# mheinz757/AgglomerationMultigrid1D

Measured on AMD Instinct MI355X. Metric: fine_level_dof_updates_per_s_per_vcycle, higher is better.
Workload: dtype f64; 1 GPU; config 3/4 hierarchy: V(3,3) cycle, alpha=2/3, DG p=3 n=2^24 -> AggDG pAgg=1 4:1 -> 2:1 -> 2:1 (4 levels), uniform mesh, Neumann/Dirichlet, CDir=1000n (north-star 1-vs-8-GPU size; config 3's own 2^22 in config3_2p22); fine_dofs=67108864, nPre=3, nPost=3, parallelism=single GPU

## Files before the change

agglomerationmultigrid1d_amd/_lib.py:

```python
import ctypes
import os
from ctypes import POINTER, c_char_p, c_double, c_int, c_int32, c_int64, c_void_p

_HERE = os.path.dirname(os.path.abspath(__file__))
LIB_PATH = os.environ.get("AGGMG_HIP_LIB") or os.path.join(_HERE, "libaggmg_hip.so")

AGGMG_OK = 0
ERR_ARGUMENT, ERR_DIMENSION, ERR_SINGULAR, ERR_HIP, ERR_UNSUPPORTED = -1, -2, -3, -4, -5
OP_STIFFNESS, OP_TRANSFER = 0, 1
OPT_SYMMETRIC_PACKING = 1
OPT_COARSE_CHUNK_LOG2 = 2
OPT_DETECT_CHAIN = 3
OPT_PAIR_LEVELS = 4
OPT_MG_CHECKPOINT = 5
OPT_SYMMETRIC_RESIDUAL = 6
OPT_OPERATOR_DICTIONARY = 7
OPT_ELEMENT_THREADS = 8
OPT_PAIR_ELEMENT_THREADS = 9
OPT_REPLAY_PRESMOOTH = 10
OPT_PATCH_MULTI = 11
OPT_CHAIN_MULTI = 12
PROFILE_NTAGS = 256
KIND_FUSED_DOWN, KIND_FUSED_UP, KIND_SMOOTH, KIND_RESIDUAL, KIND_RESTRICT, KIND_PROLONG, \
    KIND_JACOBI, KIND_BLOCK_APPLY, KIND_COARSE, KIND_FUSED_MID = range(10)
KIND_REPLAY_DOWN, KIND_REPLAY_UP = 10, 11
KIND_NAMES = ["fused_down", "fused_up", "smooth", "residual", "restrict", "prolong", "jacobi",
              "block_apply", "coarse", "fused_mid"]
COARSE_HOST_BANDED, COARSE_DEVICE_CR, COARSE_AUTO, COARSE_EXTERNAL = 0, 1, 2, 3
COARSE_DEVICE_CHAIN = 4
RESTRICT_EXPLICIT, RESTRICT_PRECONDITIONED = 0, 1
RESTRICT_PRECONDITIONED_MAX_ELEMS = 1 << 21
LEVEL_GENERIC, LEVEL_FUSED_BTD, LEVEL_FUSED_CHAIN, LEVEL_COARSEST = 0, 1, 2, 3
MAX_SWEEP_WEIGHTS = 8
FGMRES_MAX_RESTART = 64
RCCL_ID_BYTES = 128
DIST_X0_GHOSTS_VALID, DIST_OVERLAP_NEXT, DIST_GRAPH = 1, 2, 4
# ... 31 lines not shown
                              UnsupportedError)}

_P = c_void_p
_PD = POINTER(c_double)
SYMBOLS = {
    "aggmg_create": (c_int, [c_int, POINTER(_P)]),
    "aggmg_destroy": (c_int, [_P]),
    "aggmg_last_error": (c_char_p, [_P]),
    "aggmg_set_stream": (c_int, [_P, _P]),
    "aggmg_reset_stream": (c_int, [_P]),
    "aggmg_synchronize": (c_int, [_P]),
    "aggmg_set_option": (c_int, [_P, c_int, c_int]),
    "aggmg_element_thread_launches": (c_int, [_P, POINTER(c_int64)]),
    "aggmg_pair_element_thread_launches": (c_int, [_P, POINTER(c_int64)]),
    "aggmg_replay_launches": (c_int, [_P, POINTER(c_int64)]),
    "aggmg_patch_multi_launches": (c_int, [_P, POINTER(c_int64)]),
    "aggmg_chain_multi_launches": (c_int, [_P, POINTER(c_int64)]),
    "aggmg_chain_multi_tile_plan": (c_int, [c_int, c_int, c_int, c_int, c_int, POINTER(c_int), POINTER(c_int), POINTER(c_int),
                                            POINTER(c_int), POINTER(c_int)]),
    "aggmg_dev_alloc": (c_int, [_P, c_int64, POINTER(_P)]),
    "aggmg_dev_free": (c_int, [_P, _P]),
    "aggmg_memcpy_h2d": (c_int, [_P, _P, _P, c_int64]),
    "aggmg_memcpy_d2h": (c_int, [_P, _P, _P, c_int64]),
    "aggmg_csc_upload": (c_int, [_P, c_int64, c_int64, POINTER(c_int64), POINTER(c_int64), _PD,
                                 c_int, c_int, POINTER(_P)]),
    "aggmg_op_free": (c_int, [_P, _P]),
    "aggmg_op_shape": (c_int, [_P, _P, POINTER(c_int64), POINTER(c_int64), POINTER(c_int64)]),
    "aggmg_op_download": (c_int, [_P, _P, c_int, POINTER(c_int32), POINTER(c_int32), _PD]),
    "aggmg_op_release_host": (c_int, [_P, _P]),
    "aggmg_bd_sp_apply": (c_int, [_P, _P, _P, c_int, POINTER(_P)]),
# ... 156 lines not shown
```

agglomerationmultigrid1d_amd/api.py:

```python
import ctypes

import numpy as np
import scipy.sparse as sp
import scipy.sparse.linalg as spla

from . import _lib
from ._lib import (ArgumentError, DimensionMismatch, check)

_PD = ctypes.POINTER(ctypes.c_double)
_PI64 = ctypes.POINTER(ctypes.c_int64)


def _f64(x):
    return np.ascontiguousarray(x, dtype=np.float64)


def _pd(a):
    return a.ctypes.data_as(_PD)


def device_memory():
    n, b = ctypes.c_int64(), ctypes.c_int64()
    check(_lib.load().aggmg_debug_device_memory(ctypes.byref(n), ctypes.byref(b)), None)
    return n.value, b.value
# ... 31 lines not shown

    def element_thread_launches(self):
        n = ctypes.c_int64(0)
        self.check(self.lib.aggmg_element_thread_launches(self.handle, ctypes.byref(n)))
        return int(n.value)

    def pair_element_thread_launches(self):
        n = ctypes.c_int64(0)
        self.check(self.lib.aggmg_pair_element_thread_launches(self.handle, ctypes.byref(n)))
        return int(n.value)

    def replay_launches(self):
        n = ctypes.c_int64(0)
        self.check(self.lib.aggmg_replay_launches(self.handle, ctypes.byref(n)))
        return int(n.value)

    def patch_multi_launches(self):
        n = ctypes.c_int64(0)
        self.check(self.lib.aggmg_patch_multi_launches(self.handle, ctypes.byref(n)))
        return int(n.value)

    def chain_multi_launches(self):
        n = ctypes.c_int64(0)
        self.check(self.lib.aggmg_chain_multi_launches(self.handle, ctypes.byref(n)))
        return int(n.value)

    def option(self, option, default):
        return self.__dict__.get("_options", {}).get(int(option), default)

    def set_stream(self, hip_stream):
# ... 1526 lines not shown
```

agglomerationmultigrid1d_amd/csrc/aggmg_hip.hip:

```cpp
#include "internal.hpp"
#include "multi_kernels.hpp"
#include "multi_solve_kernels.hpp"
#include "pair_kernels.hpp"
#include "patch_kernels.hpp"
#include "patch_multi_kernels.hpp"
#include "elem_kernels.hpp"
#include "pair_elem_kernels.hpp"
#include "krylov_kernels.hpp"
#include "host_gmres.hpp"
#include "host_gmres_cols.hpp"

extern "C" const char* aggmg_version(void) { return "aggmg_hip 0.1 gfx950 fp64"; }

extern "C" int aggmg_debug_device_memory(int64_t* live_allocations, int64_t* live_bytes) {
  if (live_allocations) *live_allocations = DevMemLive::allocations.load();
  if (live_bytes) *live_bytes = DevMemLive::bytes.load();
  return AGGMG_OK;
}

extern "C" int aggmg_create(int device_id, aggmg_ctx** out) {
  if (!out) return fail(nullptr, AGGMG_ERR_ARGUMENT, "aggmg_create: out is NULL");
  *out = nullptr;
  int ndev = 0;
  hipError_t e = hipGetDeviceCount(&ndev);
// ... 133 lines not shown
    case AGGMG_OPT_SYMMETRIC_RESIDUAL:
      ctx->sym_residual = value != 0;
      return AGGMG_OK;
    case AGGMG_OPT_OPERATOR_DICTIONARY:
      ctx->op_dict = value != 0;
      return AGGMG_OK;
    case AGGMG_OPT_ELEMENT_THREADS:
      ctx->elem_threads = value != 0;
      return AGGMG_OK;
    case AGGMG_OPT_PAIR_ELEMENT_THREADS:
      ctx->pair_elem_threads = value != 0;
      return AGGMG_OK;
    case AGGMG_OPT_REPLAY_PRESMOOTH:
      ctx->replay_presmooth = value != 0;
      return AGGMG_OK;
    case AGGMG_OPT_PATCH_MULTI:
      ctx->patch_multi = value != 0;
      return AGGMG_OK;
    case AGGMG_OPT_CHAIN_MULTI:
      ctx->chain_multi = value != 0;
      return AGGMG_OK;
  }
  return fail(ctx, AGGMG_ERR_ARGUMENT, "aggmg_set_option: unknown option");
}

extern "C" int aggmg_synchronize(aggmg_ctx* ctx) {
  if (!ctx) return AGGMG_ERR_ARGUMENT;
  HIPCHK(hipStreamSynchronize(ctx->stream));
  return AGGMG_OK;
}
// ... 327 lines not shown
  static const int max_shift = env_int("AGGMG_AGG_ALIGN", 1) ? 8 : -1;
  return (!t.rho && t.maxagg >= 1 && t.maxagg - 1 <= max_shift) ? t.maxagg - 1 : -1;
}
static void xfer_out(FusedArgs& a, const TransferBtd& t) {
  a.lf1_out = t.lf1;
  a.mc_out = t.mc;
  a.rho_out = t.rho;
  a.par_out = t.rho ? nullptr : t.parent;
  a.first_out = t.rho ? nullptr : t.first;
  a.nec_out = t.nec;
  a.agg_shift = xfer_agg_shift(t);
}

struct FusedLaunch : FusedArgs {
  SweepWeights wts;
};

static bool elem_thread_args(const aggmg_ctx* ctx, const FusedArgs& a, bool chk, int sel_mode) {
  return ctx->elem_threads && a.lv.cls && a.lv.bsym && !a.gs && !chk && a.nsweeps >= 1 && sel_mode == 0 && !a.r_out &&
         !a.par_in && !a.par_out && !a.ld_out && (!a.lf_in || a.mc_in == 2) && (!a.lf_out || a.mc_out == 2) &&
         (!a.do_residual || a.lf_out);
}

template <int M, bool CMP>
static int launch_btd_t(aggmg_ctx* ctx, FusedLaunch a, int halo, const TileSel& sel, CgtChk* chk_io) {
  using T = BtdTile<M, CMP>;
  const bool vr = (a.lf_out || a.ld_out) && a.par_out;
  const int align = ((a.lf_out || a.ld_out) && !vr) ? a.rho_out : 1;
  if (a.gs) halo += a.nsweeps;
  if (vr && (sel.mode == 1 || sel.mode == 2))
    return fail(ctx, AGGMG_ERR_UNSUPPORTED, "tile selection on a level with agglomerates of different sizes");
  const bool chk = a.chk_part != nullptr;
  bool elem = false;
  if constexpr (M == 4 && CMP)
    elem = elem_thread_args(ctx, a, chk, sel.mode) && fused_tile_plan(kElemThreads, halo, align, vr, a.agg_shift).owned > 0;
  const FusedTilePlan plan = fused_tile_plan(elem ? kElemThreads : T::TE, halo, align, vr, a.agg_shift);
// ... 25 lines not shown
  const size_t lds = (size_t)2 * (T::TE + 2) * M * sizeof(double) +
                     (chk ? ((size_t)2 * (T::NT / 64) + (CMP ? (size_t)T::NT * T::NS * (M + 1) : 0)) * sizeof(double) : 0);
  constexpr bool kGrp = (CMP && (M == 2 || M == 4 || M == 8)) || (!CMP && (M == 2 || M == 4));
  const bool sym = kGrp && a.lv.bsym;
  constexpr bool kSres = kGrp && CMP && M <= 4;
  const bool sres = kSres && a.lv.dup && !a.gs && !chk && a.do_residual && (a.r_out || a.lf_out);
  auto go = [&](auto kern) {
    hipLaunchKernelGGL(kern, dim3((unsigned)ntiles), dim3(T::NT), lds, ctx->stream, static_cast<const FusedArgs&>(a), a.wts);
  };
  if constexpr (kGrp && CMP && M <= 4) {
    if (sym && a.lv.cls) {
      if (a.gs || chk) return fail(ctx, AGGMG_ERR_UNSUPPORTED, "internal: dictionary launch of a Gauss-Seidel / checkpoint variant");
      if (a.par_in || a.par_out || a.ld_out || (a.lf_in && a.mc_in != 2) || (a.lf_out && a.mc_out != 2))
        return fail(ctx, AGGMG_ERR_UNSUPPORTED, "internal: dictionary launch with a transfer the variant does not index by class");
      if constexpr (M == 4) {
        if (elem) {
          auto go_elem = [&](auto kern) {
            hipLaunchKernelGGL(kern, dim3((unsigned)ntiles), dim3(kElemThreads), elem_lds_bytes<M>(), ctx->stream,
                               static_cast<const FusedArgs&>(a), a.wts);
          };
          if (sres)
            go_elem(btd_elem_dict_kernel<M, true>);
          else
            go_elem(btd_elem_dict_kernel<M, false>);
          HIPCHK(hipGetLastError());
          ++ctx->elem_launches;
          return AGGMG_OK;
        }
      }
      if (sres)
// ... 93 lines not shown
  a.uc = uc;
  xfer_in(a, *l.tb);
}
static bool restrict_with_ld(const aggmg_hier* h, const Level& l) {
  return l.tb->ld && h->restriction == AGGMG_RESTRICT_PRECONDITIONED;
}
static void fused_descent(FusedArgs& a, const aggmg_hier* h, const Level& l, double* rc) {
  a.do_residual = 1;
  if (restrict_with_ld(h, l))
    a.ld_out = l.tb->ld;
  else
    a.lf_out = l.tb->lf;
  a.rc_out = rc;
  xfer_out(a, *l.tb);
}
static void fused_dictionary(FusedArgs& a, const Level& l) {
  const DictDev* d = l.dict.get();
  if (!d || a.gs || a.chk_part || a.ld_out || a.par_in || a.par_out || !a.lv.bsym) return;
  if ((a.lf_in && a.mc_in != 2) || (a.lf_out && a.mc_out != 2)) return;
  a.lv.bsym = d->bsym;
  a.lv.qrow = d->qrow;
  a.lv.qmir = d->qmir;
  a.lv.dup = d->dup;
  a.lv.corr = d->corr;
  a.lv.scol = d->scol;
  a.lv.dblk = d->dblk;
  a.lv.cls = d->cls;
  if (a.lf_in) (d->lf_unit ? a.lf1_in : a.lf_in) = d->lf;
  if (a.lf_out) (d->lf_unit ? a.lf1_out : a.lf_out) = d->lf;
}
static void fused_chk(FusedArgs& a, const CgtChk& c) {
  a.chk_sweep = c.sweep;
  a.chk_stride = c.stride;
  a.chk_final = c.final;
  a.chk_exact = c.exact;
  a.chk_part = c.part;
}

static int btd_max_sweeps(const BtdDev& b, int extra) {
  const int te = btd_tile_elems(b);
  int s = std::min(8, te / 8) - extra;
  return std::max(1, s);
// ... 1651 lines not shown
  return AGGMG_OK;
}

extern "C" int aggmg_element_thread_launches(aggmg_ctx* ctx, int64_t* count) {
  if (!ctx || !count) return fail(ctx, AGGMG_ERR_ARGUMENT, "aggmg_element_thread_launches: NULL argument");
  *count = ctx->elem_launches;
  return AGGMG_OK;
}

extern "C" int aggmg_pair_element_thread_launches(aggmg_ctx* ctx, int64_t* count) {
  if (!ctx || !count) return fail(ctx, AGGMG_ERR_ARGUMENT, "aggmg_pair_element_thread_launches: NULL argument");
  *count = ctx->pair_elem_launches;
  return AGGMG_OK;
}

extern "C" int aggmg_replay_launches(aggmg_ctx* ctx, int64_t* count) {
  if (!ctx || !count) return fail(ctx, AGGMG_ERR_ARGUMENT, "aggmg_replay_launches: NULL argument");
  *count = ctx->replay_launches;
  return AGGMG_OK;
}

extern "C" int aggmg_hier_level_dictionary(aggmg_ctx* ctx, const aggmg_hier* h, int level, int* nclasses) {
  if (!ctx || !h || !nclasses) return fail(ctx, AGGMG_ERR_ARGUMENT, "aggmg_hier_level_dictionary: NULL argument");
  if (level < 0 || level >= (int)h->lv.size()) return fail(ctx, AGGMG_ERR_ARGUMENT, "aggmg_hier_level_dictionary: level out of range");
  const Level& l = h->lv[level];
  *nclasses = l.dict ? l.dict->nclasses : (l.cdict ? l.cdict->nclasses : (l.pdict ? l.pdict->nclasses : 0));
  return AGGMG_OK;
}

extern "C" int aggmg_hier_set_sweep_weights(aggmg_ctx* ctx, aggmg_hier* h, int level, const double* pre, int npre,
// ... 152 lines not shown
  return true;
}
static int btd_replay_up(aggmg_ctx* ctx, aggmg_hier* h, const double* x0, const double* b, int nPre, int nPost, double alpha,
                         double* dst) {
  FusedLaunch a = replay_up_args(h, x0, b, nPre, nPost, alpha, dst);
  const FusedTilePlan plan = fused_tile_plan(kElemThreads, nPre + nPost, 1, false, a.agg_shift);
  if (plan.owned <= 0) return fail(ctx, AGGMG_ERR_UNSUPPORTED, "internal: replayed ascent without a tile");
  a.agg_shift = plan.agg_shift;
  a.owned = plan.owned;
  a.halo_left = plan.halo_left;
  const TileSubset sub = fused_tile_subset(a.lv.ne, plan.owned, 0, 0, 0);
  a.tile_split = sub.split;
  a.tile_skip = sub.skip;
  if (sub.ntiles == 0) return AGGMG_OK;
  ProfScope ps(ctx, AGGMG_KIND_FUSED_UP, 0);
  hipLaunchKernelGGL(btd_elem_replay_up_kernel<4>, dim3((unsigned)sub.ntiles), dim3(kElemThreads), elem_lds_bytes<4>(), ctx->stream,
                     static_cast<const FusedArgs&>(a), a.wts, nPre);
  HIPCHK(hipGetLastError());
  ++ctx->elem_launches;
  ++ctx->replay_launches;
  return AGGMG_OK;
}

static bool patch_transfer_ok(const Level& l, int residual, const TransferBtd* tout) {
  if (!l.tb) return false;
  const BtdDev& B = *l.S->patch->btd;
  TileQuery q;
  q.launch = kTileFused;
  q.te = btd_tile_elems(B);
  q.halo = residual;
  if (tout) {
    q.var_agg = tout->rho == 0;
    q.align = tout->rho ? tout->rho : 1;
    q.agg_shift = xfer_agg_shift(*tout);
// ... 2395 lines not shown
```

agglomerationmultigrid1d_amd/csrc/elem_kernels.hpp:

```cpp
#pragma once
#include <type_traits>

#include "kernels.hpp"

namespace aggmg {

typedef double elem_v2d __attribute__((ext_vector_type(2)));
__device__ __forceinline__ void elem_ld2(const double* p, double& x, double& y) {
  const elem_v2d v = *reinterpret_cast<const elem_v2d*>(p);
  x = v.x;
  y = v.y;
}
template <int M>
__host__ __device__ constexpr int elem_tri(int i, int j) {
  return i * M - (i * (i - 1)) / 2 + (j - i);
}
template <int M>
__device__ __forceinline__ double elem_sym_row_apply(const double (&tri)[M * (M + 1) / 2], int i, const double (&v)[M]) {
  double acc = 0.0;
#pragma unroll
  for (int j = 0; j < M; ++j) acc = __fma_rn(tri[i < j ? elem_tri<M>(i, j) : elem_tri<M>(j, i)], v[j], acc);
  return acc;
}
__device__ __forceinline__ void elem_group_dot4(const double (&a)[4], const double (&b)[4], double& lo, double& hi) {
// ... 367 lines not shown
    double* const op = a.u_out + e0 * M + (unsigned)(x * M);
#pragma unroll
    for (int j = 0; j < M; j += 2) {
      elem_v2d v;
      v.x = uu[j];
      v.y = uu[j + 1];
#if AGGMG_NT & 2
      __builtin_nontemporal_store(v, reinterpret_cast<elem_v2d*>(op + j));
#else
      *reinterpret_cast<elem_v2d*>(op + j) = v;
#endif
    }
  }
}

}
```

agglomerationmultigrid1d_amd/csrc/host_plan.hpp:

```cpp
#pragma once
#include <algorithm>
#include <cstddef>
#include <cstdint>
#include <vector>

namespace aggmg {

constexpr int kCrTailRows = 4096;
constexpr int kCrMaxLevels = 40;
constexpr int kCrMaxStageLevels = 12;
constexpr int kCrMaxSteps = 8;

struct CrStagePlan {
  int l0 = 0, q = 0;
  int64_t n_in = 0, n_out = 0;
  int nsteps = 0;
  int step_a[kCrMaxSteps + 1] = {0};
  int lds_off[kCrMaxSteps + 1] = {0}, lds_xoff[kCrMaxSteps + 1] = {0};
  int lds_total = 0;
  int stack_stride = 0;
  int64_t mid_off[kCrMaxSteps + 1] = {0};
  int64_t mid_total = 0;
};

// ... 409 lines not shown
  int64_t rm = W[0];
  for (int k = 0; k < nl - 1; ++k) {
    if (ratio[k] < 1) return false;
    pu[k] = std::min(rm, W[k]) - dist_sweep_reach(kind[k], nPre, k > 0);
    if (pu[k] < 1) return false;
    rm = (pu[k] - 1) / ratio[k];
  }
  int64_t v = W[nl - 1];
  for (int k = nl - 2; k >= 0; --k) {
    v = std::min(pu[k], ratio[k] * v) - dist_sweep_reach(kind[k], nPost, false);
    if (v < 0) return false;
  }
  return true;
}

}
```

agglomerationmultigrid1d_amd/csrc/internal.hpp:

```cpp
#pragma once
#include "../../include/aggmg_hip.h"

#include <hip/hip_runtime.h>

#include <algorithm>
#include <array>
#include <atomic>
#include <chrono>
#include <cmath>
#include <cstdio>
#include <cstdlib>
#include <cstring>
#include <memory>
#include <string>
#include <type_traits>
#include <vector>

#include "kernels.hpp"
#include "cr_kernels.hpp"
#include "cgt_kernels.hpp"

using namespace aggmg;

struct aggmg_ctx;
// ... 28 lines not shown
  int device = 0;
  hipStream_t own_stream = nullptr;
  hipStream_t stream = nullptr;
  std::string err;
  bool sym_packing = true;
  int cr_max_q = 12;
  bool detect_chain = true;
  bool mg_checkpoint = [] { const char* e = std::getenv("AGGMG_MG_CHECKPOINT"); return !(e && e[0] == '0'); }();
  bool pair_levels = [] { const char* e = std::getenv("AGGMG_PAIR"); return !(e && e[0] == '0'); }();
  bool sym_residual = [] { const char* e = std::getenv("AGGMG_SYM_RESIDUAL"); return !(e && e[0] == '0'); }();
  bool op_dict = [] { const char* e = std::getenv("AGGMG_OP_DICT"); return !(e && e[0] == '0'); }();
  bool elem_threads = [] { const char* e = std::getenv("AGGMG_ELEM_THREADS"); return !(e && e[0] == '0'); }();
  int64_t elem_launches = 0;
  bool pair_elem_threads = [] { const char* e = std::getenv("AGGMG_PAIR_ELEM_THREADS"); return !(e && e[0] == '0'); }();
  int64_t pair_elem_launches = 0;
  bool replay_presmooth = [] { const char* e = std::getenv("AGGMG_REPLAY_PRESMOOTH"); return !(e && e[0] == '0'); }();
  int64_t replay_launches = 0;
  bool patch_multi = [] { const char* e = std::getenv("AGGMG_PATCH_MULTI"); return e && e[0] == '1'; }();
  int64_t patch_multi_launches = 0;
  bool chain_multi = [] { const char* e = std::getenv("AGGMG_CHAIN_MULTI"); return e && e[0] == '1'; }();
  int64_t chain_multi_launches = 0;
  int profiling = 0;
  std::vector<ProfEvent> prof;
  std::vector<hipEvent_t> ev_pool;
  WorkVectors<kScratchSlots> scratch;
  WorkVectors<kSolvSlots> solv;
  DevArray<double> solv_part, solv_sc;
  DevArray<double> cols_part, cols_sc;
  DevArray<int> cols_map;
  int64_t cols_cap = 0;
// ... 123 lines not shown
  DevArray<double> lf;
  DevArray<double> lf1;
  DevArray<double> ld;
  DevArray<int32_t> parent;
  DevArray<int32_t> first;
  int maxagg = 0;
};

struct DictDev {
  int nclasses = 0;
  DevArray<uint16_t> cls;
  DevArray<double> bsym, qrow, qmir, dup, scol, dblk;
  DevArray<uint32_t> corr;
  DevArray<double> lf;
  bool lf_unit = false;
};

struct PairDictDev {
  int nclasses = 0;
  DevArray<uint16_t> cls;
  DevArray<double> bsym, sup, sback, sub, dblk;
  DevArray<double> lf;
  bool lf_unit = false;
  DevArray<double> rec;
};

struct TransferCgt {
  int type = 0, mc = 0, rho = 1;
  int64_t nec = 0;
  DevArray<double> l, lp;
// ... 255 lines not shown
```

agglomerationmultigrid1d_amd/csrc/setup.hip:

```cpp
#include <functional>

#include <hipcub/hipcub.hpp>

#include "internal.hpp"
#include "setup_kernels.hpp"
#include "pair_elem_kernels.hpp"

namespace {

inline unsigned grid_for(int64_t n) { return (unsigned)((n + kSetupThreads - 1) / kSetupThreads); }

struct Flags {
  DevArray<int> d;
  int n = 0;
  int init(aggmg_ctx* ctx, int count) {
    n = count;
    return d.alloc(ctx, count, true);
  }
  int read(aggmg_ctx* ctx, int* host) {
    HIPCHK(hipMemcpyAsync(host, d, n * sizeof(int), hipMemcpyDeviceToHost, ctx->stream));
    HIPCHK(hipStreamSynchronize(ctx->stream));
    return AGGMG_OK;
  }
  int clear(aggmg_ctx* ctx) {
// ... 539 lines not shown
  const int T = m * (m + 1) / 2;
  auto d = std::make_unique<DictDev>();
  d->lf_unit = t.lf1 != nullptr;
  DictFields F(b.ne);
  F.add(b.bsym, &d->bsym, T);
  F.add(b.qrow, &d->qrow, m);
  F.add(b.qrow, &d->qmir, m, true);
  if (b.dup) {
    F.add(b.dup, &d->dup, T);
    F.add(b.corr, &d->corr, m);
  }
  F.add(b.scol, &d->scol, m);
  F.add(b.dblk, &d->dblk, m * m);
  F.add(t.lf1 ? t.lf1 : t.lf, &d->lf, m * (t.lf1 ? 1 : 2));
  CHECK(dict_build(ctx, F, &d->cls, &d->nclasses));
  if (d->nclasses > 0) *out = std::move(d);
  return AGGMG_OK;
}

int setup_pair_dictionary(aggmg_ctx* ctx, const BtdDev& b, const TransferBtd& t, std::unique_ptr<PairDictDev>* out) {
  out->reset();
  const int m = b.m;
  if (!(!b.cmp && m == 2 && b.bsym && b.sup && b.sub && b.dblk) || b.ne < 1) return AGGMG_OK;
  if (!(t.rho > 0 && t.mc == 2 && t.lf)) return AGGMG_OK;
  auto d = std::make_unique<PairDictDev>();
  d->lf_unit = t.lf1 != nullptr;
  DictFields F(b.ne);
  F.add(b.bsym, &d->bsym, m * (m + 1) / 2);
  F.add(b.sup, &d->sup, m * m);
  F.add(b.sup, &d->sback, m * m, true);
// ... 623 lines not shown
```

include/aggmg_hip.h:

```cpp
#ifndef AGGMG_HIP_H
#define AGGMG_HIP_H

#include <stdint.h>

#ifdef __cplusplus
extern "C" {
#endif

#define AGGMG_OK 0
#define AGGMG_ERR_ARGUMENT (-1)
#define AGGMG_ERR_DIMENSION (-2)
#define AGGMG_ERR_SINGULAR (-3)
#define AGGMG_ERR_HIP (-4)
#define AGGMG_ERR_UNSUPPORTED (-5)

typedef struct aggmg_ctx aggmg_ctx;
typedef struct aggmg_op aggmg_op;
typedef struct aggmg_smoother aggmg_smoother;
typedef struct aggmg_hier aggmg_hier;

int aggmg_create(int device_id, aggmg_ctx** out);
int aggmg_destroy(aggmg_ctx* ctx);
const char* aggmg_last_error(aggmg_ctx* ctx);
int aggmg_set_stream(aggmg_ctx* ctx, void* hip_stream);
int aggmg_reset_stream(aggmg_ctx* ctx);
int aggmg_synchronize(aggmg_ctx* ctx);
#define AGGMG_OPT_SYMMETRIC_PACKING 1
#define AGGMG_OPT_COARSE_CHUNK_LOG2 2
#define AGGMG_OPT_DETECT_CHAIN 3
#define AGGMG_OPT_PAIR_LEVELS 4
#define AGGMG_OPT_MG_CHECKPOINT 5
#define AGGMG_OPT_SYMMETRIC_RESIDUAL 6
#define AGGMG_OPT_OPERATOR_DICTIONARY 7
#define AGGMG_OPT_ELEMENT_THREADS 8
#define AGGMG_OPT_PAIR_ELEMENT_THREADS 9
#define AGGMG_OPT_REPLAY_PRESMOOTH 10
#define AGGMG_OPT_PATCH_MULTI 11
#define AGGMG_OPT_CHAIN_MULTI 12
int aggmg_set_option(aggmg_ctx* ctx, int option, int value);
int aggmg_element_thread_launches(aggmg_ctx* ctx, int64_t* count);
int aggmg_pair_element_thread_launches(aggmg_ctx* ctx, int64_t* count);
int aggmg_replay_launches(aggmg_ctx* ctx, int64_t* count);
int aggmg_patch_multi_launches(aggmg_ctx* ctx, int64_t* count);
int aggmg_chain_multi_launches(aggmg_ctx* ctx, int64_t* count);
int aggmg_chain_multi_tile_plan(int m, int nsweeps, int restrict_kind, int rho, int kb, int* tile_blocks, int* owned,
                                int* halo_left, int* halo_right, int* max_sweeps);
int aggmg_dev_alloc(aggmg_ctx* ctx, int64_t nbytes, void** out);
int aggmg_dev_free(aggmg_ctx* ctx, void* ptr);
int aggmg_memcpy_h2d(aggmg_ctx* ctx, void* dst_dev, const void* src_host, int64_t nbytes);
int aggmg_memcpy_d2h(aggmg_ctx* ctx, void* dst_host, const void* src_dev, int64_t nbytes);
int aggmg_host_register(aggmg_ctx* ctx, void* ptr, int64_t nbytes);
int aggmg_host_unregister(aggmg_ctx* ctx, void* ptr);
int aggmg_host_alloc(aggmg_ctx* ctx, int64_t nbytes, void** out);
int aggmg_host_free(aggmg_ctx* ctx, void* ptr);
// ... 243 lines not shown
```

Measured before the change: 467.7 billion DoF-updates/s.

## Stage per-class element records in LDS for element-thread fused kernels

```diff
diff --git a/agglomerationmultigrid1d_amd/_lib.py b/agglomerationmultigrid1d_amd/_lib.py
--- a/agglomerationmultigrid1d_amd/_lib.py
+++ b/agglomerationmultigrid1d_amd/_lib.py
@@ -20,6 +20,7 @@
 OPT_REPLAY_PRESMOOTH = 10
 OPT_PATCH_MULTI = 11
 OPT_CHAIN_MULTI = 12
+OPT_ELEMENT_RECORDS_LDS = 13
 PROFILE_NTAGS = 256
 KIND_FUSED_DOWN, KIND_FUSED_UP, KIND_SMOOTH, KIND_RESIDUAL, KIND_RESTRICT, KIND_PROLONG, \
     KIND_JACOBI, KIND_BLOCK_APPLY, KIND_COARSE, KIND_FUSED_MID = range(10)
@@ -81,6 +82,9 @@
     "aggmg_element_thread_launches": (c_int, [_P, POINTER(c_int64)]),
     "aggmg_pair_element_thread_launches": (c_int, [_P, POINTER(c_int64)]),
     "aggmg_replay_launches": (c_int, [_P, POINTER(c_int64)]),
+    "aggmg_element_record_lds_launches": (c_int, [_P, POINTER(c_int64)]),
+    "aggmg_element_record_lds_cap": (c_int, [_P, POINTER(c_int), POINTER(c_int)]),
+    "aggmg_element_record_pack": (c_int, [c_int, _P, _P, _P, _P, _P, _P, c_int, _P, POINTER(c_int)]),
     "aggmg_patch_multi_launches": (c_int, [_P, POINTER(c_int64)]),
     "aggmg_chain_multi_launches": (c_int, [_P, POINTER(c_int64)]),
     "aggmg_chain_multi_tile_plan": (c_int, [c_int, c_int, c_int, c_int, c_int, POINTER(c_int), POINTER(c_int), POINTER(c_int),
diff --git a/agglomerationmultigrid1d_amd/api.py b/agglomerationmultigrid1d_amd/api.py
--- a/agglomerationmultigrid1d_amd/api.py
+++ b/agglomerationmultigrid1d_amd/api.py
@@ -69,6 +69,16 @@
         n = ctypes.c_int64(0)
         self.check(self.lib.aggmg_replay_launches(self.handle, ctypes.byref(n)))
         return int(n.value)
+
+    def element_record_lds_launches(self):
+        n = ctypes.c_int64(0)
+        self.check(self.lib.aggmg_element_record_lds_launches(self.handle, ctypes.byref(n)))
+        return int(n.value)
+
+    def element_record_lds_cap(self):
+        c, m = ctypes.c_int(0), ctypes.c_int(0)
+        self.check(self.lib.aggmg_element_record_lds_cap(self.handle, ctypes.byref(c), ctypes.byref(m)))
+        return int(c.value), int(m.value)
 
     def patch_multi_launches(self):
         n = ctypes.c_int64(0)
diff --git a/agglomerationmultigrid1d_amd/csrc/aggmg_hip.hip b/agglomerationmultigrid1d_amd/csrc/aggmg_hip.hip
--- a/agglomerationmultigrid1d_amd/csrc/aggmg_hip.hip
+++ b/agglomerationmultigrid1d_amd/csrc/aggmg_hip.hip
@@ -171,6 +171,11 @@
     case AGGMG_OPT_REPLAY_PRESMOOTH:
       ctx->replay_presmooth = value != 0;
       return AGGMG_OK;
+    case AGGMG_OPT_ELEMENT_RECORDS_LDS:
+      if (value < 0 || value > kElemRecMaxClasses)
+        return fail(ctx, AGGMG_ERR_ARGUMENT, "aggmg_set_option: AGGMG_OPT_ELEMENT_RECORDS_LDS takes 0 .. " + std::to_string(kElemRecMaxClasses));
+      ctx->elem_rec_cap = value;
+      return AGGMG_OK;
     case AGGMG_OPT_PATCH_MULTI:
       ctx->patch_multi = value != 0;
       return AGGMG_OK;
@@ -528,12 +533,16 @@
 
 struct FusedLaunch : FusedArgs {
   SweepWeights wts;
+  ElemRecTab rec = {nullptr, 0};
 };
 
 static bool elem_thread_args(const aggmg_ctx* ctx, const FusedArgs& a, bool chk, int sel_mode) {
   return ctx->elem_threads && a.lv.cls && a.lv.bsym && !a.gs && !chk && a.nsweeps >= 1 && sel_mode == 0 && !a.r_out &&
          !a.par_in && !a.par_out && !a.ld_out && (!a.lf_in || a.mc_in == 2) && (!a.lf_out || a.mc_out == 2) &&
          (!a.do_residual || a.lf_out);
+}
+static bool elem_record_args(const aggmg_ctx* ctx, const FusedLaunch& a) {
+  return a.rec.rec && a.rec.nclasses >= 1 && a.rec.nclasses <= ctx->elem_rec_cap && (!a.do_residual || (a.lv.dup && a.lv.corr));
 }
 
 template <int M, bool CMP>
@@ -589,6 +598,20 @@
       if (a.par_in || a.par_out || a.ld_out || (a.lf_in && a.mc_in != 2) || (a.lf_out && a.mc_out != 2))
         return fail(ctx, AGGMG_ERR_UNSUPPORTED, "internal: dictionary launch with a transfer the variant does not index by class");
       if constexpr (M == 4) {
+        if (elem && elem_record_args(ctx, a)) {
+          auto go_rec = [&](auto kern) {
+            hipLaunchKernelGGL(kern, dim3((unsigned)ntiles), dim3(kElemThreads), elem_rec_lds_bytes<M>(a.rec.nclasses), ctx->stream,
+                               static_cast<const FusedArgs&>(a), a.wts, a.rec);
+          };
+          if (a.do_residual)
+            go_rec(btd_elem_rec_kernel<M, true>);
+          else
+            go_rec(btd_elem_rec_kernel<M, false>);
+          HIPCHK(hipGetLastError());
+          ++ctx->elem_launches;
+          ++ctx->elem_rec_launches;
+          return AGGMG_OK;
+        }
         if (elem) {
           auto go_elem = [&](auto kern) {
             hipLaunchKernelGGL(kern, dim3((unsigned)ntiles), dim3(kElemThreads), elem_lds_bytes<M>(), ctx->stream,
@@ -712,7 +735,7 @@
   a.rc_out = rc;
   xfer_out(a, *l.tb);
 }
-static void fused_dictionary(FusedArgs& a, const Level& l) {
+static void fused_dictionary(FusedLaunch& a, const Level& l) {
   const DictDev* d = l.dict.get();
   if (!d || a.gs || a.chk_part || a.ld_out || a.par_in || a.par_out || !a.lv.bsym) return;
   if ((a.lf_in && a.mc_in != 2) || (a.lf_out && a.mc_out != 2)) return;
@@ -724,6 +747,7 @@
   a.lv.scol = d->scol;
   a.lv.dblk = d->dblk;
   a.lv.cls = d->cls;
+  if (d->rec) a.rec = ElemRecTab{d->rec, d->nclasses};
   if (a.lf_in) (d->lf_unit ? a.lf1_in : a.lf_in) = d->lf;
   if (a.lf_out) (d->lf_unit ? a.lf1_out : a.lf_out) = d->lf;
 }
@@ -2405,6 +2429,27 @@
   return AGGMG_OK;
 }
 
+extern "C" int aggmg_element_record_lds_launches(aggmg_ctx* ctx, int64_t* count) {
+  if (!ctx || !count) return fail(ctx, AGGMG_ERR_ARGUMENT, "aggmg_element_record_lds_launches: NULL argument");
+  *count = ctx->elem_rec_launches;
+  return AGGMG_OK;
+}
+
+extern "C" int aggmg_element_record_lds_cap(aggmg_ctx* ctx, int* cap, int* max_cap) {
+  if (!ctx || !cap) return fail(ctx, AGGMG_ERR_ARGUMENT, "aggmg_element_record_lds_cap: NULL argument");
+  *cap = ctx->elem_rec_cap;
+  if (max_cap) *max_cap = kElemRecMaxClasses;
+  return AGGMG_OK;
+}
+
+extern "C" int aggmg_element_record_pack(int nclasses, const double* bsym, const double* qrow, const double* qmir, const double* dup,
+                                         const uint32_t* corr, const double* lf, int lf_unit, double* rec, int* words) {
+  if (words) *words = kElemRecWords;
+  if (nclasses < 0 || (nclasses > 0 && (!bsym || !qrow || !qmir || !lf || !rec || !dup != !corr))) return AGGMG_ERR_ARGUMENT;
+  elem_record_pack(nclasses, bsym, qrow, qmir, dup, corr, lf, lf_unit != 0, rec);
+  return AGGMG_OK;
+}
+
 extern "C" int aggmg_replay_launches(aggmg_ctx* ctx, int64_t* count) {
   if (!ctx || !count) return fail(ctx, AGGMG_ERR_ARGUMENT, "aggmg_replay_launches: NULL argument");
   *count = ctx->replay_launches;
@@ -2587,10 +2632,16 @@
   a.tile_skip = sub.skip;
   if (sub.ntiles == 0) return AGGMG_OK;
   ProfScope ps(ctx, AGGMG_KIND_FUSED_UP, 0);
-  hipLaunchKernelGGL(btd_elem_replay_up_kernel<4>, dim3((unsigned)sub.ntiles), dim3(kElemThreads), elem_lds_bytes<4>(), ctx->stream,
-                     static_cast<const FusedArgs&>(a), a.wts, nPre);
+  const bool rec = elem_record_args(ctx, a);
+  if (rec)
+    hipLaunchKernelGGL(btd_elem_rec_replay_up_kernel<4>, dim3((unsigned)sub.ntiles), dim3(kElemThreads),
+                       elem_rec_lds_bytes<4>(a.rec.nclasses), ctx->stream, static_cast<const FusedArgs&>(a), a.wts, nPre, a.rec);
+  else
+    hipLaunchKernelGGL(btd_elem_replay_up_kernel<4>, dim3((unsigned)sub.ntiles), dim3(kElemThreads), elem_lds_bytes<4>(), ctx->stream,
+                       static_cast<const FusedArgs&>(a), a.wts, nPre);
   HIPCHK(hipGetLastError());
   ++ctx->elem_launches;
+  if (rec) ++ctx->elem_rec_launches;
   ++ctx->replay_launches;
   return AGGMG_OK;
 }
diff --git a/agglomerationmultigrid1d_amd/csrc/elem_kernels.hpp b/agglomerationmultigrid1d_amd/csrc/elem_kernels.hpp
--- a/agglomerationmultigrid1d_amd/csrc/elem_kernels.hpp
+++ b/agglomerationmultigrid1d_amd/csrc/elem_kernels.hpp
@@ -1,6 +1,7 @@
 #pragma once
 #include <type_traits>
 
+#include "host_plan.hpp"
 #include "kernels.hpp"
 
 namespace aggmg {
@@ -405,4 +406,352 @@
   }
 }
 
-}
+struct ElemRecTab {
+  const double* rec;
+  int nclasses;
+};
+template <int M>
+constexpr size_t elem_rec_lds_bytes(int nclasses) {
+  return elem_lds_bytes<M>() + (size_t)nclasses * kElemRecWords * sizeof(double);
+}
+
+constexpr int kElemRecStage = (kElemRecMaxClasses * (kElemRecWords / 2) + kElemThreads - 1) / kElemThreads;
+__device__ __forceinline__ void elem_rec_fetch(const ElemRecTab& t, int x, elem_v2d (&v)[kElemRecStage]) {
+  const int n = t.nclasses * (kElemRecWords / 2);
+#pragma unroll
+  for (int k = 0; k < kElemRecStage; ++k) {
+    const int i = x + k * kElemThreads;
+    if (k == 0 || k * kElemThreads < n) v[k] = reinterpret_cast<const elem_v2d*>(t.rec)[i < n ? i : n - 1];
+  }
+}
+__device__ __forceinline__ void elem_rec_store(double* tab, const ElemRecTab& t, int x, const elem_v2d (&v)[kElemRecStage]) {
+  const int n = t.nclasses * (kElemRecWords / 2);
+#pragma unroll
+  for (int k = 0; k < kElemRecStage; ++k) {
+    const int i = x + k * kElemThreads;
+    if (i < n) reinterpret_cast<elem_v2d*>(tab)[i] = v[k];
+  }
+}
+
+template <class V>
+__device__ __forceinline__ void elem_rec_pin(V& v) {
+  asm volatile("" : "+v"(v));
+}
+template <int M>
+__device__ __forceinline__ void elem_rec_pin_all(unsigned& ce, double (&bb)[M], double (&uu)[M], double& ucx, double& ucy) {
+  elem_rec_pin(ce);
+#pragma unroll
+  for (int j = 0; j < M; ++j) elem_rec_pin(bb[j]);
+#pragma unroll
+  for (int j = 0; j < M; ++j) elem_rec_pin(uu[j]);
+  elem_rec_pin(ucx);
+  elem_rec_pin(ucy);
+}
+
+template <int M>
+struct ElemRecStencil {
+  double q[M], pc[M], br[M];
+  __device__ __forceinline__ void load(const double* rec, int r_sup) {
+#pragma unroll
+    for (int j = 0; j < M; j += 2) elem_ld2(rec + kElemRecQrow + j, q[j], q[j + 1]);
+#pragma unroll
+    for (int j = 0; j < M; j += 2) elem_ld2(rec + kElemRecPcol + j, pc[j], pc[j + 1]);
+#pragma unroll
+    for (int i = 0; i < M; ++i) br[i] = rec[kElemRecBsym + (i < r_sup ? elem_tri<M>(i, r_sup) : elem_tri<M>(r_sup, i))];
+  }
+};
+template <int M>
+__device__ __forceinline__ void elem_rec_g(const double* rec, const double (&bb)[M], double (&g)[M]) {
+  constexpr int T = M * (M + 1) / 2;
+  double tri[T];
+#pragma unroll
+  for (int k = 0; k < T; k += 2) elem_ld2(rec + kElemRecBsym + k, tri[k], tri[k + 1]);
+#pragma unroll
+  for (int i = 0; i < M; ++i) g[i] = elem_sym_row_apply<M>(tri, i, bb);
+}
+template <int M, bool ADD>
+__device__ __forceinline__ void elem_rec_sweep(const ElemRecStencil<M>& st, double*& cur, double*& nxt, int x, int c_sub,
+                                               double w, bool valid, const double (&g)[M], double (&uu)[M],
+                                               const double* luc) {
+  constexpr int S = kElemThreads + 2;
+  const double um = cur[c_sub * S + x - 1];
+  double up[M];
+#pragma unroll
+  for (int j = 0; j < M; ++j) up[j] = cur[j * S + x + 1];
+  double dlo, dhi;
+  elem_group_dot4(st.q, up, dlo, dhi);
+#pragma unroll
+  for (int i = 0; i < M; ++i) {
+    double acc = __fma_rn(-st.pc[i], um, g[i]);
+    acc = __fma_rn(-st.br[i], i < 2 ? dlo : dhi, acc);
+    double un = __fma_rn(w, __dadd_rn(acc, -uu[i]), uu[i]);
+    if constexpr (ADD) un = __dadd_rn(un, luc[i]);
+    if (!valid) un = 0.0;
+    uu[i] = un;
+    nxt[i * S + x] = un;
+  }
+  __syncthreads();
+  double* t = cur;
+  cur = nxt;
+  nxt = t;
+}
+__device__ __forceinline__ void elem_rec_st_iterate(double* op, const double (&uu)[4]) {
+#pragma unroll
+  for (int j = 0; j < 4; j += 2) {
+    elem_v2d v;
+    v.x = uu[j];
+    v.y = uu[j + 1];
+#if AGGMG_NT & 2
+    __builtin_nontemporal_store(v, reinterpret_cast<elem_v2d*>(op + j));
+#else
+    *reinterpret_cast<elem_v2d*>(op + j) = v;
+#endif
+  }
+}
+
+template <int M, bool RES>
+__global__ __launch_bounds__(kElemThreads) void btd_elem_rec_kernel(FusedArgs a, SweepWeights wts, ElemRecTab t) {
+  static_assert(M == 4, "the element-thread kernel's block size");
+  constexpr int TE = kElemThreads;
+  constexpr int S = TE + 2;
+  constexpr int T = M * (M + 1) / 2;
+  extern __shared__ double lds[];
+  double* cur = lds + 1;
+  double* nxt = lds + M * S + 1;
+  double* const tab = lds + 2 * M * S;
+
+  const int x = threadIdx.x;
+  const int64_t ne = a.lv.ne;
+  const int64_t e0 = fused_tile(a) * a.owned - a.halo_left;
+  const int own0 = a.halo_left, own1 = a.halo_left + a.owned;
+  const int64_t rem = ne - 1 - e0;
+  if (rem < 0) return;
+  const int xlo = e0 < 0 ? (int)-e0 : 0, xhi = rem < TE - 1 ? (int)rem : TE - 1;
+  const bool valid = x >= xlo && x <= xhi;
+  const bool own = valid && x >= own0 && x < own1;
+  const unsigned xc = (unsigned)(x < xlo ? xlo : x > xhi ? xhi : x);
+
+  elem_v2d tv[kElemRecStage];
+  elem_rec_fetch(t, x, tv);
+  const bool pro = a.lf_in != nullptr;
+  unsigned ce = (a.lv.cls + e0)[xc];
+  double bb[M], uu[M];
+  {
+    const double* const bp = a.b + e0 * M + xc * M;
+    const double* const up = (a.u_in ? a.u_in : a.b) + e0 * M + xc * M;
+#pragma unroll
+    for (int j = 0; j < M; j += 2) elem_ld2(bp + j, bb[j], bb[j + 1]);
+#pragma unroll
+    for (int j = 0; j < M; j += 2) elem_ld2(up + j, uu[j], uu[j + 1]);
+  }
+  double ucx = 0.0, ucy = 0.0;
+  if (pro) {
+    const int64_t J = ne <= 0x7fffffff ? (int64_t)((unsigned)(e0 + xc) / (unsigned)a.rho_in) : (e0 + xc) / a.rho_in;
+    elem_ld2(a.uc + J * 2, ucx, ucy);
+  }
+  elem_rec_store(tab, t, x, tv);
+  if (x < 4 * M) {
+    const int j = x & (M - 1), w = x / M;
+    (w & 2 ? nxt : cur)[j * S + (w & 1 ? TE : -1)] = 0.0;
+  }
+  __syncthreads();
+  elem_rec_pin_all<M>(ce, bb, uu, ucx, ucy);
+  if (!a.u_in) {
+#pragma unroll
+    for (int j = 0; j < M; ++j) uu[j] = 0.0;
+  }
+
+  const double* const rec = tab + ce * kElemRecWords;
+  if (pro) {
+#pragma unroll
+    for (int j = 0; j < M; ++j) {
+      double lx, ly;
+      elem_ld2(rec + kElemRecLf + 2 * j, lx, ly);
+      uu[j] = __dadd_rn(uu[j], __fma_rn(lx, ucx, __dmul_rn(ly, ucy)));
+    }
+  }
+  if (!valid) {
+#pragma unroll
+    for (int j = 0; j < M; ++j) {
+      uu[j] = 0.0;
+      bb[j] = 0.0;
+    }
+  }
+  double g[M];
+  elem_rec_g<M>(rec, bb, g);
+#pragma unroll
+  for (int i = 0; i < M; ++i) cur[i * S + x] = uu[i];
+  const int c_sub = a.lv.c_sub, r_sup = a.lv.r_sup;
+  ElemRecStencil<M> st;
+  st.load(rec, r_sup);
+  __syncthreads();
+
+  for (int sw = 0; sw < a.nsweeps; ++sw)
+    elem_rec_sweep<M, false>(st, cur, nxt, x, c_sub, wts.w[(unsigned)sw], valid, g, uu, nullptr);
+
+  if (a.u_out && own) elem_rec_st_iterate(a.u_out + e0 * M + (unsigned)(x * M), uu);
+  if constexpr (RES) {
+    double D[M][M], sc[M];
+    {
+      double du[T];
+#pragma unroll
+      for (int k = 0; k < T; k += 2) elem_ld2(rec + kElemRecDup + k, du[k], du[k + 1]);
+      const uint4 w4 = *reinterpret_cast<const uint4*>(rec + kElemRecCorr);
+      const uint32_t w[M] = {w4.x, w4.y, w4.z, w4.w};
+#pragma unroll
+      for (int j = 0; j < M; j += 2) elem_ld2(rec + kElemRecQmir + j, sc[j], sc[j + 1]);
+      bool esc = false;
+#pragma unroll
+      for (int i = 0; i < M; ++i) {
+#pragma unroll
+        for (int j = 0; j < M; ++j) {
+          if (j >= i) {
+            D[i][j] = du[elem_tri<M>(i, j)];
+          } else {
+            const int d = (int)(int8_t)(w[i] >> (8 * j));
+            D[i][j] = sym_residual_decode(du[elem_tri<M>(j, i)], d);
+            esc |= d == kSymResidualEscape;
+          }
+        }
+        const int dc = (int)(int8_t)(w[i] >> 24);
+        sc[i] = sym_residual_decode(sc[i], dc);
+        esc |= dc == kSymResidualEscape;
+      }
+      if (__builtin_expect(own && esc, 0)) {
+#pragma unroll
+        for (int i = 0; i < M; ++i) {
+#pragma unroll
+          for (int j = 0; j < i; ++j)
+            if ((int)(int8_t)(w[i] >> (8 * j)) == kSymResidualEscape) D[i][j] = a.lv.dblk[((int64_t)ce * M + i) * M + j];
+          if ((int)(int8_t)(w[i] >> 24) == kSymResidualEscape) sc[i] = a.lv.scol[(int64_t)ce * M + i];
+        }
+      }
+    }
+    double rr[M];
+    {
+      const double um = cur[c_sub * S + x - 1];
+      double up[M];
+#pragma unroll
+      for (int j = 0; j < M; ++j) up[j] = cur[j * S + x + 1];
+      double dlo, dhi;
+      elem_group_dot4(st.q, up, dlo, dhi);
+#pragma unroll
+      for (int i = 0; i < M; ++i) {
+        double s = __fma_rn(sc[i], um, 0.0);
+#pragma unroll
+        for (int j = 0; j < M; ++j) s = __fma_rn(D[i][j], uu[j], s);
+        if (i == r_sup) s = __dadd_rn(s, i < 2 ? dlo : dhi);
+        rr[i] = own ? __dadd_rn(bb[i], -s) : 0.0;
+      }
+    }
+    __syncthreads();
+#pragma unroll
+    for (int i = 0; i < M; ++i) {
+      double lx, ly;
+      elem_ld2(rec + kElemRecLf + 2 * i, lx, ly);
+      nxt[i * S + x] = own ? __dmul_rn(lx, rr[i]) : 0.0;
+      cur[i * S + x] = own ? __dmul_rn(ly, rr[i]) : 0.0;
+    }
+    __syncthreads();
+    const int rho = a.rho_out;
+    const int ncoarse = a.owned / rho;
+    const int64_t J0 = fused_tile(a) * ncoarse;
+    for (int k2 = x; k2 < ncoarse * 2; k2 += TE) {
+      const int Jl = k2 >> 1, c = k2 & 1;
+      const int64_t J = J0 + Jl;
+      if (J >= a.nec_out) continue;
+      const double* pr = (c ? cur : nxt) + a.halo_left + Jl * rho;
+      double acc = 0.0;
+      for (int k = 0; k < rho; ++k) {
+#pragma unroll
+        for (int j = 0; j < M; ++j) acc = __dadd_rn(acc, pr[j * S + k]);
+      }
+      a.rc_out[J * 2 + c] = acc;
+    }
+  }
+}
+
+template <int M>
+__global__ __launch_bounds__(kElemThreads) void btd_elem_rec_replay_up_kernel(FusedArgs a, SweepWeights wts, int npre, ElemRecTab t) {
+  static_assert(M == 4, "the element-thread kernel's block size");
+  constexpr int TE = kElemThreads;
+  constexpr int S = TE + 2;
+  extern __shared__ double lds[];
+  double* cur = lds + 1;
+  double* nxt = lds + M * S + 1;
+  double* const tab = lds + 2 * M * S;
+
+  const int x = threadIdx.x;
+  const int64_t ne = a.lv.ne;
+  const int64_t e0 = fused_tile(a) * a.owned - a.halo_left;
+  const int own0 = a.halo_left, own1 = a.halo_left + a.owned;
+  const int64_t rem = ne - 1 - e0;
+  if (rem < 0) return;
+  const int xlo = e0 < 0 ? (int)-e0 : 0, xhi = rem < TE - 1 ? (int)rem : TE - 1;
+  const bool valid = x >= xlo && x <= xhi;
+  const bool own = valid && x >= own0 && x < own1;
+  const unsigned xc = (unsigned)(x < xlo ? xlo : x > xhi ? xhi : x);
+
+  elem_v2d tv[kElemRecStage];
+  elem_rec_fetch(t, x, tv);
+  unsigned ce = (a.lv.cls + e0)[xc];
+  double bb[M], uu[M];
+  {
+    const double* const bp = a.b + e0 * M + xc * M;
+    const double* const up = (a.u_in ? a.u_in : a.b) + e0 * M + xc * M;
+#pragma unroll
+    for (int j = 0; j < M; j += 2) elem_ld2(bp + j, bb[j], bb[j + 1]);
+#pragma unroll
+    for (int j = 0; j < M; j += 2) elem_ld2(up + j, uu[j], uu[j + 1]);
+  }
+  double ucx, ucy;
+  {
+    const int64_t J = ne <= 0x7fffffff ? (int64_t)((unsigned)(e0 + xc) / (unsigned)a.rho_in) : (e0 + xc) / a.rho_in;
+    elem_ld2(a.uc + J * 2, ucx, ucy);
+  }
+  elem_rec_store(tab, t, x, tv);
+  if (x < 4 * M) {
+    const int j = x & (M - 1), w = x / M;
+    (w & 2 ? nxt : cur)[j * S + (w & 1 ? TE : -1)] = 0.0;
+  }
+  __syncthreads();
+  elem_rec_pin_all<M>(ce, bb, uu, ucx, ucy);
+  if (!a.u_in) {
+#pragma unroll
+    for (int j = 0; j < M; ++j) uu[j] = 0.0;
+  }
+
+  const double* const rec = tab + ce * kElemRecWords;
+  double luc[M];
+#pragma unroll
+  for (int j = 0; j < M; ++j) {
+    double lx, ly;
+    elem_ld2(rec + kElemRecLf + 2 * j, lx, ly);
+    luc[j] = __fma_rn(lx, ucx, __dmul_rn(ly, ucy));
+  }
+  if (!valid) {
+#pragma unroll
+    for (int j = 0; j < M; ++j) {
+      uu[j] = 0.0;
+      bb[j] = 0.0;
+    }
+  }
+  double g[M];
+  elem_rec_g<M>(rec, bb, g);
+#pragma unroll
+  for (int i = 0; i < M; ++i) cur[i * S + x] = uu[i];
+  const int c_sub = a.lv.c_sub, r_sup = a.lv.r_sup;
+  ElemRecStencil<M> st;
+  st.load(rec, r_sup);
+  __syncthreads();
+
+  for (int sw = 0; sw < npre - 1; ++sw)
+    elem_rec_sweep<M, false>(st, cur, nxt, x, c_sub, wts.w[(unsigned)sw], valid, g, uu, nullptr);
+  elem_rec_sweep<M, true>(st, cur, nxt, x, c_sub, wts.w[(unsigned)(npre - 1)], valid, g, uu, luc);
+  for (int sw = npre; sw < a.nsweeps; ++sw)
+    elem_rec_sweep<M, false>(st, cur, nxt, x, c_sub, wts.w[(unsigned)sw], valid, g, uu, nullptr);
+
+  if (own) elem_rec_st_iterate(a.u_out + e0 * M + (unsigned)(x * M), uu);
+}
+
+}
diff --git a/agglomerationmultigrid1d_amd/csrc/host_plan.hpp b/agglomerationmultigrid1d_amd/csrc/host_plan.hpp
--- a/agglomerationmultigrid1d_amd/csrc/host_plan.hpp
+++ b/agglomerationmultigrid1d_amd/csrc/host_plan.hpp
@@ -1,7 +1,9 @@
 #pragma once
 #include <algorithm>
+#include <cmath>
 #include <cstddef>
 #include <cstdint>
+#include <cstring>
 #include <vector>
 
 namespace aggmg {
@@ -447,4 +449,38 @@
   return true;
 }
 
-}
+constexpr int kElemRecWords = 42;
+constexpr int kElemRecBsym = 0, kElemRecPcol = 10, kElemRecQrow = 14, kElemRecQmir = 18, kElemRecDup = 22, kElemRecCorr = 32,
+              kElemRecLf = 34;
+static_assert(kElemRecWords % 2 == 0 && kElemRecPcol % 2 == 0 && kElemRecQrow % 2 == 0 && kElemRecQmir % 2 == 0 &&
+                  kElemRecDup % 2 == 0 && kElemRecCorr % 2 == 0 && kElemRecLf % 2 == 0,
+              "the groups of a record are read 16 bytes at a time");
+#ifndef AGGMG_ELEM_REC_MAX_CLASSES
+#define AGGMG_ELEM_REC_MAX_CLASSES 32
+#endif
+constexpr int kElemRecMaxClasses = AGGMG_ELEM_REC_MAX_CLASSES;
+inline void elem_record_pack(int nclasses, const double* bsym, const double* qrow, const double* qmir, const double* dup,
+                             const uint32_t* corr, const double* lf, bool lf_unit, double* rec) {
+  constexpr int M = 4, T = 10;
+  auto tri = [](int i, int j) { return i * M - (i * (i - 1)) / 2 + (j - i); };
+  for (int c = 0; c < nclasses; ++c) {
+    double* r = rec + (size_t)c * kElemRecWords;
+    for (int k = 0; k < kElemRecWords; ++k) r[k] = 0.0;
+    for (int k = 0; k < T; ++k) r[kElemRecBsym + k] = bsym[c * T + k];
+    for (int i = 0; i < M; ++i) {
+      double acc = 0.0;
+      for (int j = 0; j < M; ++j) acc = std::fma(bsym[c * T + (i < j ? tri(i, j) : tri(j, i))], qmir[c * M + j], acc);
+      r[kElemRecPcol + i] = acc;
+      r[kElemRecQrow + i] = qrow[c * M + i];
+      r[kElemRecQmir + i] = qmir[c * M + i];
+      r[kElemRecLf + 2 * i] = lf_unit ? 1.0 : lf[(c * M + i) * 2];
+      r[kElemRecLf + 2 * i + 1] = lf_unit ? lf[c * M + i] : lf[(c * M + i) * 2 + 1];
+    }
+    if (dup && corr) {
+      for (int k = 0; k < T; ++k) r[kElemRecDup + k] = dup[c * T + k];
+      std::memcpy(r + kElemRecCorr, corr + c * M, M * sizeof(uint32_t));
+    }
+  }
+}
+
+}
diff --git a/agglomerationmultigrid1d_amd/csrc/internal.hpp b/agglomerationmultigrid1d_amd/csrc/internal.hpp
--- a/agglomerationmultigrid1d_amd/csrc/internal.hpp
+++ b/agglomerationmultigrid1d_amd/csrc/internal.hpp
@@ -66,6 +66,8 @@
   int64_t elem_launches = 0;
   bool pair_elem_threads = [] { const char* e = std::getenv("AGGMG_PAIR_ELEM_THREADS"); return !(e && e[0] == '0'); }();
   int64_t pair_elem_launches = 0;
+  int elem_rec_cap = [] { const char* e = std::getenv("AGGMG_ELEM_RECORDS_LDS"); return (e && e[0] == '0') ? 0 : kElemRecMaxClasses; }();
+  int64_t elem_rec_launches = 0;
   bool replay_presmooth = [] { const char* e = std::getenv("AGGMG_REPLAY_PRESMOOTH"); return !(e && e[0] == '0'); }();
   int64_t replay_launches = 0;
   bool patch_multi = [] { const char* e = std::getenv("AGGMG_PATCH_MULTI"); return e && e[0] == '1'; }();
@@ -219,6 +221,7 @@
   DevArray<uint32_t> corr;
   DevArray<double> lf;
   bool lf_unit = false;
+  DevArray<double> rec;
 };
 
 struct PairDictDev {
diff --git a/agglomerationmultigrid1d_amd/csrc/setup.hip b/agglomerationmultigrid1d_amd/csrc/setup.hip
--- a/agglomerationmultigrid1d_amd/csrc/setup.hip
+++ b/agglomerationmultigrid1d_amd/csrc/setup.hip
@@ -577,6 +577,29 @@
   F.add(b.dblk, &d->dblk, m * m);
   F.add(t.lf1 ? t.lf1 : t.lf, &d->lf, m * (t.lf1 ? 1 : 2));
   CHECK(dict_build(ctx, F, &d->cls, &d->nclasses));
+  if (m == 4 && d->nclasses > 0 && d->nclasses <= kElemRecMaxClasses) {
+    const int nc = d->nclasses, nl = d->lf_unit ? m : 2 * m;
+    std::vector<double> hb((size_t)T * nc), hq((size_t)m * nc), hm((size_t)m * nc), hd(b.dup ? (size_t)T * nc : 0), hl((size_t)nl * nc);
+    std::vector<uint32_t> hc(b.dup ? (size_t)m * nc : 0);
+    std::vector<double> rec((size_t)nc * kElemRecWords);
+    auto down = [&](auto& v, const auto* src) {
+      return hipMemcpyAsync(v.data(), src, v.size() * sizeof(v[0]), hipMemcpyDeviceToHost, ctx->stream);
+    };
+    HIPCHK(down(hb, d->bsym.get()));
+    HIPCHK(down(hq, d->qrow.get()));
+    HIPCHK(down(hm, d->qmir.get()));
+    if (b.dup) {
+      HIPCHK(down(hd, d->dup.get()));
+      HIPCHK(down(hc, d->corr.get()));
+    }
+    HIPCHK(down(hl, d->lf.get()));
+    HIPCHK(hipStreamSynchronize(ctx->stream));
+    elem_record_pack(nc, hb.data(), hq.data(), hm.data(), b.dup ? hd.data() : nullptr, b.dup ? hc.data() : nullptr, hl.data(),
+                     d->lf_unit, rec.data());
+    CHECK(d->rec.alloc(ctx, (int64_t)rec.size()));
+    HIPCHK(hipMemcpyAsync(d->rec, rec.data(), rec.size() * sizeof(double), hipMemcpyHostToDevice, ctx->stream));
+    HIPCHK(hipStreamSynchronize(ctx->stream));
+  }
   if (d->nclasses > 0) *out = std::move(d);
   return AGGMG_OK;
 }
diff --git a/include/aggmg_hip.h b/include/aggmg_hip.h
--- a/include/aggmg_hip.h
+++ b/include/aggmg_hip.h
@@ -37,7 +37,12 @@
 #define AGGMG_OPT_REPLAY_PRESMOOTH 10
 #define AGGMG_OPT_PATCH_MULTI 11
 #define AGGMG_OPT_CHAIN_MULTI 12
+#define AGGMG_OPT_ELEMENT_RECORDS_LDS 13
 int aggmg_set_option(aggmg_ctx* ctx, int option, int value);
+int aggmg_element_record_lds_launches(aggmg_ctx* ctx, int64_t* count);
+int aggmg_element_record_lds_cap(aggmg_ctx* ctx, int* cap, int* max_cap);
+int aggmg_element_record_pack(int nclasses, const double* bsym, const double* qrow, const double* qmir, const double* dup,
+                              const uint32_t* corr, const double* lf, int lf_unit, double* rec, int* words);
 int aggmg_element_thread_launches(aggmg_ctx* ctx, int64_t* count);
 int aggmg_pair_element_thread_launches(aggmg_ctx* ctx, int64_t* count);
 int aggmg_replay_launches(aggmg_ctx* ctx, int64_t* count);
```

After: 528.9 billion DoF-updates/s (median of 6 runs). 1.13x the previous value.
